# deemoe404/rmcv

Hardware: AMD Instinct MI355X
Metric: frames/sec (1280x1024 BGR) armour detect (higher is better)
Workload: dtype u8

## Files before the change

### rmcv_amd/csrc/device_fit.h

```cpp
#pragma once
#include <hip/hip_runtime.h>
#include <float.h>

#include "../../include/rmcv_abi.h"
#include "pinned_math.h"
#include "device_eig3.h"

namespace rmcv {

#define RMCV_PI 3.1415926535897932384626433832795

__device__ __forceinline__ double dabs(double x) { return __builtin_fabs(x); }
__device__ __forceinline__ double dsqrt(double x) { return ::sqrt(x); }

__device__ __forceinline__ double lane_get(double reg, int idx)
{
    const unsigned long long u = (unsigned long long)__double_as_longlong(reg);
    const unsigned lo = (unsigned)__builtin_amdgcn_readlane((int)(unsigned)u, idx);
    const unsigned hi = (unsigned)__builtin_amdgcn_readlane((int)(unsigned)(u >> 32), idx);
    return __longlong_as_double((long long)(((unsigned long long)hi << 32) | lo));
}
struct LaneRef {
    double* reg;
    int idx, lane;
// ... 384 lines not shown
    LaneMat3& V = E.V;
#else
    LaneMat3 H(lane), V(lane);
    LaneVec d(lane), e(lane);
#pragma unroll
    for (int i = 0; i < 3; i++)
#pragma unroll
        for (int j = 0; j < 3; j++) H[i][j] = M[i][j];
    eig_orthes(H, V, lane);
    eig_hqr2(H, V, d, e);
#endif
    const double d0 = d.get(0), d1 = d.get(1), d2 = d.get(2);
    int i0 = 0, i1 = 1, i2 = 2;
    double e0 = d0, e1 = d1;
    if (e0 < d1) { i0 = 1; i1 = 0; e0 = d1; e1 = d0; }
    if (e1 < d2) {
        i2 = i1;
        if (e0 < d2) { i1 = i0; i0 = 2; }
        else { i1 = 2; }
    }
    const int idx[3] = {i0, i1, i2};
#pragma unroll
    for (int i = 0; i < 3; i++) {
        eval[i] = d.get(idx[i]);
#pragma unroll
        for (int j = 0; j < 3; j++) evec[i][j] = lane_get(V.reg, 3 * j + idx[i]);
    }
}

template <int K>
__device__ __forceinline__ void jacobi_sym(LaneVec& A_, LaneVec& lam, LaneVec& V_)
{
#ifdef RMCV_JACOBI_PLAIN
    double A[K * K], V[K * K];
#pragma unroll
    for (int i = 0; i < K * K; i++) A[i] = A_.get(i);
#else
    LaneVec& A = A_;
    LaneVec& V = V_;
#endif
#pragma unroll
    for (int i = 0; i < K; i++)
#pragma unroll
        for (int j = 0; j < K; j++) V[i * K + j] = (i == j) ? 1.0 : 0.0;
#pragma unroll 1
    for (int sweep = 0; sweep < 60; sweep++) {
        double off = 0.0;
#pragma unroll
        for (int p = 0; p < K; p++)
#pragma unroll
            for (int q = p + 1; q < K; q++) off += dabs(A[p * K + q]);
        if (off == 0.0) break;
#pragma unroll
        for (int p = 0; p < K; p++)
#pragma unroll
            for (int q = p + 1; q < K; q++) {
                double apq = A[p * K + q];
                if (apq == 0.0) continue;
                double app = A[p * K + p], aqq = A[q * K + q];
                if (dabs(apq) < 1e-300 || dabs(apq) <= 1.1102230246251565e-16 * 1e-3 * dsqrt(dabs(app * aqq))) {
                    A[p * K + q] = 0.0;
                    A[q * K + p] = 0.0;
                    continue;
                }
                double theta = (aqq - app) / (2.0 * apq);
                double t = 1.0 / (dabs(theta) + dsqrt(theta * theta + 1.0));
                if (theta < 0) t = -t;
                double c = 1.0 / dsqrt(t * t + 1.0);
                double s = t * c;
                A[p * K + p] = app - t * apq;
                A[q * K + q] = aqq + t * apq;
                A[p * K + q] = 0.0;
                A[q * K + p] = 0.0;
#pragma unroll
                for (int r = 0; r < K; r++) {
                    if (r != p && r != q) {
                        double arp = A[r * K + p], arq = A[r * K + q];
                        double nrp = c * arp - s * arq;
                        double nrq = s * arp + c * arq;
                        A[r * K + p] = nrp;
                        A[p * K + r] = nrp;
                        A[r * K + q] = nrq;
                        A[q * K + r] = nrq;
                    }
                    double vrp = V[r * K + p], vrq = V[r * K + q];
                    V[r * K + p] = c * vrp - s * vrq;
                    V[r * K + q] = s * vrp + c * vrq;
                }
            }
    }
#ifdef RMCV_JACOBI_PLAIN
#pragma unroll
    for (int i = 0; i < K * K; i++) {
        A_[i] = A[i];
        V_[i] = V[i];
    }
#endif
#pragma unroll
    for (int i = 0; i < K; i++) lam[i] = (double)A[i * K + i];
}

struct NormalFac {
    LaneVec lam, V;
    int k, use;
    __device__ __forceinline__ explicit NormalFac(int lane) : lam(lane), V(lane), k(0), use(0) {}
};

template <int K>
__device__ __forceinline__ void normal_factor(LaneVec& A, NormalFac& F, double* wmax, double* wmin)
{
    F.k = K;
    jacobi_sym<K>(A, F.lam, F.V);
    double wsum = 0, mx = 0, mn = 0;
#pragma unroll
    for (int i = 0; i < K; i++) {
        const double li = F.lam[i];
        const double wi = li > 0 ? dsqrt(li) : 0.0;
        wsum += wi;
        if (i == 0 || wi > mx) mx = wi;
        if (i == 0 || wi < mn) mn = wi;
    }
    const double thr = 2.0 * DBL_EPSILON * wsum;
    F.use = 0;
#pragma unroll
    for (int i = 0; i < K; i++) {
        const double li = F.lam[i];
        const double wi = li > 0 ? dsqrt(li) : 0.0;
        F.use |= (wi > thr ? 1 : 0) << i;
    }
    *wmax = mx;
    *wmin = mn;
}
// ... 300 lines not shown
```

### rmcv_amd/csrc/k_contours.hip

```cpp
#include "contours_device.h"

namespace rmcv {

#define KC_KERNEL k_contours_w8
#define KC_THREADS 512
#include "k_contours_kernel.inc"
#undef KC_KERNEL
#undef KC_THREADS

static_assert(sizeof(ContoursLds) >= (CT_THREADS_MAX / 64) * sizeof(WaveLds), "the fit rows reuse the contour tables");

static hipError_t launch_contours_w8(const Geom& g, const Bufs& b, const Limits& lim, const SparseTail& X, int flags, const SparseSched& Q, int grid,
                                     SparseLds lds, hipStream_t s)
{
    static bool attr_set[MAX_DEVICES] = {};
    if (!attr_set[g.device]) {
        hipError_t e = hipFuncSetAttribute(reinterpret_cast<const void*>(k_contours_w8), hipFuncAttributeMaxDynamicSharedMemorySize,
                                           (int)lds_bytes(CT_MAXH));
        if (e != hipSuccess) return e;
        attr_set[g.device] = true;
    }
    return launch(k_contours_w8, dim3(grid), dim3(512), sparse_lds(lds, lds_bytes(g.h)), s, b.bits, b.rowmask, g.h, b.lab, b.neg, g.w,
                       g.h, g.ww, g.prow, g.plane_pitch, b.points, b.cont_start, b.cont_len, b.n_contours, b.n_points, b.status,
                       lim.max_contours, lim.max_points, flags, b.elig, b.n_elig, b.slot_kind, X, b.visit_xy, b.mid, b.mid_stride,
                       b.mid_slot_cap, Q, lds_rows_cap(g.h));
}

static hipError_t launch_contours_x(const Geom& g, const Bufs& b, const Limits& lim, const SparseTail& X, const RunPlan& plan, hipStream_t s,
                                    bool* lean)
{
    SparseSched Q;
    Q.order = b.frame_order;
    const SparseLaunches L = resolve_sparse({plan.form, plan.sparse_waves, X.fused != 0, X.C.enabled != 0, g.contour_tier, b.mid != nullptr,
                                             g.h <= CT_MAXH && g.ww <= 32, plan.pixel_ws != 0});
    if (lean) *lean = L.n == 1 && L.l[0].kernel == SPARSE_W_LEAN;
    for (int i = 0; i < L.n; i++) {
        const SparseLaunch& l = L.l[i];
        const hipError_t e = (l.kernel == SPARSE_W8 ? launch_contours_w8 : l.kernel == SPARSE_W4 ? launch_contours_w4 : launch_contours_lean)(
            g, b, lim, X, l.flags, Q, g.n_frames, l.lds, s);
        if (e != hipSuccess) return e;
    }
    return hipSuccess;
}

hipError_t launch_contours(const Geom& g, const Bufs& b, const Limits& lim, hipStream_t s)
{
    SparseTail X;
    memset(&X, 0, sizeof(X));
    return launch_contours_x(g, b, lim, X, RunPlan{0, 0, 8, SPARSE_STANDARD}, s, nullptr);
}

hipError_t launch_sparse(const Geom& g, const Bufs& b, const Limits& lim, const rmcv_params& p, bool pairs, bool identity, const RunPlan& plan,
                         hipStream_t s, bool* lean)
{
    SparseTail X;
    memset(&X, 0, sizeof(X));
    X.fused = 1;
    X.G = {p.tilt_max, p.ratio_lo, p.ratio_hi, p.area_lo, p.area_hi, g.overloads};
    X.slot_ell = b.slot_ell;
    FitTail& T = X.T;
    T.blobs = b.blobs;
    T.blob_src = b.blob_src;
    T.ellipses = b.ellipses;
    T.neg_idx = b.neg_idx;
    T.n_blobs = b.n_blobs;
    T.n_neg = b.n_neg;
    T.status = b.status;
    T.armours = b.armours;
    T.n_armours = b.n_armours;
    T.max_blobs = lim.max_blobs;
    T.max_armours = lim.max_armours;
    T.enemy = p.camp;
    T.enemy_tab = enemy_table(g, b);
    T.do_pairs = pairs ? 1 : 0;
    T.angle_diff_max = p.angle_diff_max;
    T.shear_max = p.shear_max;
    T.length_ratio_max = p.length_ratio_max;
    T.ov = g.overloads;
    if (identity && pairs) X.C = classify_args(g, b);
    return launch_contours_x(g, b, lim, X, plan, s, lean);
}

__device__ __forceinline__ void export_lists(const ExportArgs& a, int gtid, int nthreads)
{
    if (gtid < 12 && a.hdr_src[gtid]) a.hdr_dst[gtid] = *a.hdr_src[gtid];
    for (int k = 0; k < a.n_sec; k++) {
        const ExportSec& e = a.sec[k];
        int n = e.count ? e.count[0] + e.count_add : e.max_elems;
        n = n < 0 ? 0 : (n > e.max_elems ? e.max_elems : n);
        const int ndw = n * (e.elem_bytes >> 2);
        const uint32_t* src = static_cast<const uint32_t*>(e.src);
// ... 114 lines not shown
```

### rmcv_amd/csrc/k_contours_kernel.inc

```
#define CT_THREADS KC_THREADS
#ifndef RMCV_KC_ATTR
#define RMCV_KC_ATTR
#endif
__global__ __launch_bounds__(CT_THREADS) RMCV_KC_ATTR void KC_KERNEL(const uint64_t* __restrict__ bits, const uint32_t* __restrict__ rowmasks,
                                                        int rm_pitch, uint64_t* lab, uint64_t* neg, int w, int h, int ww, int prow,
                                                        int64_t plane_pitch, rmcv_point* points, int32_t* cont_start,
                                                        int32_t* cont_len, int32_t* n_contours, int32_t* n_points,
                                                        int32_t* status, int max_contours, int max_points, int force_literal,
                                                        int32_t* __restrict__ elig, int32_t* __restrict__ n_elig,
                                                        int32_t* __restrict__ slot_kind, SparseTail X, uint32_t* __restrict__ visit_xy,
                                                        uint8_t* __restrict__ mid_base, int64_t mid_stride, int mid_slot_cap, SparseSched Q, int rows_cap)
{
    extern __shared__ unsigned long long smem_raw[];
#ifndef RMCV_KC_PRIO
#define RMCV_KC_PRIO 3
#endif
    __builtin_amdgcn_s_setprio(RMCV_KC_PRIO);
    ContoursLds& S = *reinterpret_cast<ContoursLds*>(smem_raw);
    const RowTabs RT = row_tabs(smem_raw, rows_cap);
    const int tid = threadIdx.x, lane = tid & 63, wave = tid >> 6;
    enum { FL_COMPLEX = 1, FL_MID = 2 };
    const int f = Q.order ? Q.order[blockIdx.x] : (int)blockIdx.x;
#ifdef RMCV_PROFILE_HANDOVER
    const long long th0_ = wall_clock64(), th1_ = th0_;
#endif
    const bool defer_mid = (force_literal & 4) != 0, deferred_only = (force_literal & 8) != 0;
    force_literal &= 3;
    if (deferred_only && status[f] != RMCV_FRAME_DEFERRED_) return;
    const uint64_t* F = bits + (int64_t)f * plane_pitch;
    uint64_t* LAB = lab + (int64_t)f * plane_pitch;
    uint64_t* NEG = neg + (int64_t)f * plane_pitch;
    rmcv_point* pts = points + (int64_t)f * max_points;
    int32_t* cs = cont_start + (int64_t)f * max_contours;
// ... 220 lines not shown
    const int32_t* el = elig + (int64_t)f * max_contours;
    uint16_t* const w_len = S.n_b;
    uint16_t* const w_idx = S.n_d;
    uint16_t* const w_sorted = S.n_a;
    const uint32_t* const w_off = S.w_off;
    const uint32_t* const w_cnt = S.w_cnt;
    static_assert(KEPT_CAP <= NN_CAP, "the work list fits the node tables");
    for (int e = tid; e < ne; e += CT_THREADS) {
        int len;
        if (complex) {
            const int k = el[e];
            len = cl[k];
            w_idx[e] = (uint16_t)k;
        } else len = (int)w_cnt[e];
        w_len[e] = (uint16_t)(len > 65535 ? 65535 : len);
    }
    if (tid == 0) S.wnext = 0;
    __syncthreads();
    for (int e = tid; e < ne; e += CT_THREADS) {
        const int len = w_len[e];
        int rank = 0;
        for (int j = 0; j < ne; j++) rank += (w_len[j] > len) || (w_len[j] == len && j < e);
        w_sorted[rank] = (uint16_t)e;
    }
    __syncthreads();
    {
        static_assert(offsetof(ContoursLds, n_a) >= (CT_THREADS_MAX / 64) * sizeof(WaveLds), "the work list must outlive the tables");
        static_assert(offsetof(ContoursLds, w_off) >= (CT_THREADS_MAX / 64) * sizeof(WaveLds), "... and so must its LDS copies of starts / lengths");
        WaveLds& L = reinterpret_cast<WaveLds*>(smem_raw)[wave];
        for (;;) {
            const int got = atomicAdd(lane == 0 ? &S.wnext : &S.sink[lane], lane == 0 ? 1 : 0);
            const int e = __shfl(got, 0);
            if (e >= ne_all) break;
            if (!complex) {
                const int pos = w_sorted[e];
                fit_contour_slot_at(f, (int)w_idx[pos], nc, pts, (int)w_off[pos], (int)w_cnt[pos], max_contours, max_points, X.G, slot_kind,
                                    X.slot_ell, L, lane);
            } else {
                const int k = e < ne ? (int)w_idx[w_sorted[e]] : el[e];
                fit_contour_slot(f, k, nc, pts, cs, cl, max_contours, max_points, X.G, slot_kind, X.slot_ell, L, lane);
            }
        }
    }
    __syncthreads();
#if defined(RMCV_PROFILE) || defined(RMCV_PROFILE_HANDOVER)
    const long long tt1_ = wall_clock64();
#endif
    if (wave == 0) {
        const FitTail& T = X.T;
        const int enemy = tail_enemy(T, f);
        const int np = blob_compact_frame(f, lane, slot_kind, X.slot_ell, nc, max_contours, enemy, T.blobs, T.blob_src, T.ellipses,
                                          T.neg_idx, T.n_blobs, T.n_neg, T.status, T.max_blobs);
        if (T.do_pairs) {
            __threadfence_block();
            armours_frame(f, lane, T.blobs, np, T.max_blobs, T.angle_diff_max, T.shear_max, T.length_ratio_max, enemy, T.armours,
                          T.n_armours, T.status, T.max_armours, T.ov);
        }
    }
#ifdef RMCV_PROFILE
    __syncthreads();
    if (tid == 0 && blockIdx.x < 2) printf("[tail b%d] eligible %d of %d contours: fits %.1f us, compaction + pairing %.1f us\n", (int)blockIdx.x, ne_all, nc, (tt1_ - tt0_) / 100.0, (wall_clock64() - tt1_) / 100.0);
#endif
#ifdef RMCV_PROFILE_HANDOVER
    __syncthreads();
    if (tid == 0)
        printf("[sp] %d %lld %lld %lld | %.1f %.1f %.1f %.1f %.1f | elig %d\n", f, th0_, th1_, (long long)wall_clock64(), (t_[1] - t_[0]) / 100.0,
               (t_[2] - t_[1]) / 100.0, (tt0_ - t_[2]) / 100.0, (tt1_ - tt0_) / 100.0, (wall_clock64() - tt1_) / 100.0, ne_all);
#endif
#ifndef KC_NO_CLASSIFY
    if (X.C.enabled) {
        __threadfence_block();
        __syncthreads();
        constexpr int NW = CT_THREADS / 64;
        static_assert((CT_THREADS_MAX / 64) * sizeof(WaveLds) + NW * (NFEAT * sizeof(float) + 32 * sizeof(double)) <= sizeof(ContoursLds), "feature rows fit");
// ... 12 lines not shown
```

### rmcv_amd/csrc/k_contours_w4.hip

```cpp
#include "contours_device.h"

#include <algorithm>

namespace rmcv {

#define KC_KERNEL k_contours_w4
#define KC_THREADS 256
#include "k_contours_kernel.inc"
#undef KC_KERNEL
#undef KC_THREADS

hipError_t launch_contours_w4(const Geom& g, const Bufs& b, const Limits& lim, const SparseTail& X, int flags, const SparseSched& Q, int grid,
                              SparseLds lds, hipStream_t s)
{
    static bool attr_set[MAX_DEVICES] = {};
    if (!attr_set[g.device]) {
        hipError_t e = hipFuncSetAttribute(reinterpret_cast<const void*>(k_contours_w4), hipFuncAttributeMaxDynamicSharedMemorySize,
                                           (int)std::max(lds_bytes(CT_MAXH), LDS_ONE_PER_CU_BYTES));
        if (e != hipSuccess) return e;
        attr_set[g.device] = true;
    }
    return launch(k_contours_w4, dim3(grid), dim3(256), sparse_lds(lds, lds_bytes(g.h)), s, b.bits, b.rowmask, g.h, b.lab, b.neg, g.w,
                       g.h, g.ww, g.prow, g.plane_pitch, b.points, b.cont_start, b.cont_len, b.n_contours, b.n_points, b.status,
                       lim.max_contours, lim.max_points, flags, b.elig, b.n_elig, b.slot_kind, X, b.visit_xy, b.mid, b.mid_stride,
                       b.mid_slot_cap, Q, lds_rows_cap(g.h));
}

}
```

### rmcv_amd/csrc/k_detect.hip

```cpp
#include "device_hull.h"
#include "wave_detect.h"

namespace rmcv {

static constexpr int FIT_CHUNKS = 4;
__global__ __launch_bounds__(256) void k_fit(const rmcv_point* __restrict__ points, const int32_t* __restrict__ cont_start,
                                            const int32_t* __restrict__ cont_len, const int32_t* __restrict__ n_contours,
                                            int max_contours, int max_points, float tilt_max, float ratio_lo, float ratio_hi,
                                            double area_lo, double area_hi, int32_t* __restrict__ slot_kind,
                                            rmcv_rrect* __restrict__ slot_ell, const int32_t* __restrict__ elig,
                                            const int32_t* __restrict__ n_elig, int ov)
{
    __shared__ WaveLds lds[4];
    __builtin_amdgcn_s_setprio(3);
    const int f = blockIdx.x, lane = threadIdx.x & 63, wave = threadIdx.x >> 6;
    WaveLds& L = lds[wave];
    const int n = n_contours[f];
    const rmcv_point* pts = points + (int64_t)f * max_points;
    const int32_t* cs = cont_start + (int64_t)f * max_contours;
    const int32_t* cl = cont_len + (int64_t)f * max_contours;
    const int ne = n_elig[f];
    const FitGates G = {tilt_max, ratio_lo, ratio_hi, area_lo, area_hi, ov};
    for (int e = blockIdx.y * 4 + wave; e < ne; e += 4 * gridDim.y)
        fit_contour_slot(f, elig[(int64_t)f * max_contours + e], n, pts, cs, cl, max_contours, max_points, G, slot_kind, slot_ell, L, lane);
}

struct MatchArgs {
    float min_ratio, max_ratio, tilt_angle, min_area, max_area;
    int fit_ellipse, mode;
    int ov;
    int wcap, hcap, ccap;
    int pass;
    const uint8_t* frames;
    int64_t frame_pitch;
    int stride;
    const rmcv_point* win_eff;
};

static constexpr int MATCH_CHUNKS = 16;
static constexpr int MATCH_DEFERRED = 0x100;
__global__ __launch_bounds__(64) void k_match(const rmcv_point* __restrict__ points, const int32_t* __restrict__ cont_start,
                                             const int32_t* __restrict__ cont_len, const int32_t* __restrict__ n_contours,
                                             int max_contours, int max_points, MatchArgs A, int32_t* __restrict__ slot_kind,
                                             rmcv_rrect* __restrict__ slot_ell, const int32_t* __restrict__ elig,
                                             const int32_t* __restrict__ n_elig, int32_t* __restrict__ status)
{
    extern __shared__ unsigned long long match_smem[];
    __builtin_amdgcn_s_setprio(3);
    const int f = blockIdx.x, lane = threadIdx.x;
    WaveLds& L = *reinterpret_cast<WaveLds*>(match_smem);
    HullLds H;
    hull_lds_carve(reinterpret_cast<unsigned char*>(match_smem) + sizeof(WaveLds), A.wcap, A.hcap, A.ccap, H);
    const bool final_pass = A.pass == 1 || A.mode == 1;
    const int n = n_contours[f];
    const rmcv_point* pts = points + (int64_t)f * max_points;
    const int32_t* cs = cont_start + (int64_t)f * max_contours;
    const int32_t* cl = cont_len + (int64_t)f * max_contours;
// ... 281 lines not shown
```

### rmcv_amd/csrc/wave_detect.h

```cpp
#pragma once
#include "device_classify.h"
#include "device_fit.h"
#include "rmcv_internal.h"

namespace rmcv {

__device__ __forceinline__ int lanes_below(uint64_t m, int lane) { return __popcll(m & ((1ull << lane) - 1)); }

struct WaveLds {
    double rows[64][6];
    double terms[64];
    double dm[32];
};

__device__ __forceinline__ double wave_sum_f64(double v)
{
    for (int d = 32; d >= 1; d >>= 1) v += __shfl_xor(v, d);
    return v;
}
__device__ __forceinline__ long long wave_sum_i64(long long v)
{
    for (int d = 32; d >= 1; d >>= 1) v += __shfl_xor(v, d);
    return v;
}

template <typename F>
__device__ __forceinline__ double seq_sum_terms(int n, int lane, WaveLds& L, F term)
{
    double s = 0;
    for (int base = 0; base < n; base += 64) {
        const int i = base + lane;
        const double t = i < n ? term(i) : 0.0;
        const int m = n - base < 64 ? n - base : 64;
        if (m == 64) {
#pragma unroll
            for (int j = 0; j < 64; j++) s += lane_get(t, j);
        } else {
            for (int j = 0; j < m; j++) s += lane_get(t, j);
        }
    }
    return s;
}

template <typename F0, typename F1>
__device__ __forceinline__ void seq_sum_terms2(int n, int lane, F0 term0, F1 term1, double* s0_, double* s1_)
{
    double s0 = 0, s1 = 0;
    for (int base = 0; base < n; base += 64) {
        const int i = base + lane;
        const double t0 = i < n ? term0(i) : 0.0, t1 = i < n ? term1(i) : 0.0;
        const int m = n - base < 64 ? n - base : 64;
        if (m == 64) {
#pragma unroll
            for (int j = 0; j < 64; j++) { s0 += lane_get(t0, j); s1 += lane_get(t1, j); }
        } else {
            for (int j = 0; j < m; j++) { s0 += lane_get(t0, j); s1 += lane_get(t1, j); }
        }
    }
    *s0_ = s0;
    *s1_ = s1;
}

template <int NR, typename F>
__device__ __forceinline__ double seq_sum_products_two(int n, int lane, WaveLds& L, int ns, int la, int lb, F make_row )
{
    double acc = 0;
    const int half = lane >> 5, l5 = lane & 31;
    for (int base = 0; base < n; base += 32) {
        const int i = base + l5;
        if (i < n) {
            double r[NR];
            make_row(i, half, r);
#pragma unroll
            for (int k = 0; k < NR; k++) L.rows[lane][k] = r[k];
        }
        __builtin_amdgcn_wave_barrier();
        const int m = n - base < 32 ? n - base : 32;
        if (l5 < ns) {
            const int r0 = half * 32;
#pragma unroll 8
            for (int j = 0; j < m; j++) acc += L.rows[r0 + j][la] * L.rows[r0 + j][lb];
        }
        __builtin_amdgcn_wave_barrier();
    }
    return acc;
}

template <int NR, typename F>
__device__ __forceinline__ double seq_sum_products(int n, int lane, WaveLds& L, int ns, int la, int lb, double konst, F make_row)
{
    double acc = 0;
    for (int base = 0; base < n; base += 64) {
        const int i = base + lane;
        if (i < n) {
            double r[NR];
            make_row(i, r);
#pragma unroll
            for (int k = 0; k < NR; k++) L.rows[lane][k] = r[k];
        }
        __builtin_amdgcn_wave_barrier();
        const int m = n - base < 64 ? n - base : 64;
        if (lane < ns) {
            if (lb >= 0) {
#pragma unroll 8
                for (int j = 0; j < m; j++) acc += L.rows[j][la] * L.rows[j][lb];
            } else {
#pragma unroll 8
                for (int j = 0; j < m; j++) acc += L.rows[j][la] * konst;
            }
        }
        __builtin_amdgcn_wave_barrier();
    }
    return acc;
}

template <int K, typename F>
__device__ __forceinline__ void par_sum_products(int n, int lane, double konst, double* out, F make_row)
{
    constexpr int NT = K * (K + 1) / 2, NS = NT + K;
    double acc[NS];
#pragma unroll
    for (int e = 0; e < NS; e++) acc[e] = 0.0;
#pragma unroll 1
    for (int i = lane; i < n; i += 64) {
        double row[K];
        make_row(i, row);
        int e = 0;
#pragma unroll
        for (int a = 0; a < K; a++)
#pragma unroll
            for (int b = a; b < K; b++, e++) acc[e] += row[a] * row[b];
#pragma unroll
        for (int a = 0; a < K; a++) acc[NT + a] += row[a] * konst;
    }
    for (int d = 32; d >= 1; d >>= 1) {
        double o[NS];
#pragma unroll
        for (int e = 0; e < NS; e++) o[e] = __shfl_xor(acc[e], d);
#pragma unroll
        for (int e = 0; e < NS; e++) acc[e] += o[e];
    }
#pragma unroll
    for (int e = 0; e < NS; e++) out[e] = acc[e];
}

__device__ __forceinline__ void tri_index(int e, int k, int* a, int* b)
{
    int r = 0, rem = e;
    while (r < k && rem >= k - r) { rem -= k - r; r++; }
    *a = r;
    *b = r + rem;
}

template <int K, typename F>
__device__ __forceinline__ void normal_refine(NormalFac& Fac, int n, int lane, double bconst, double* x , F make_row)
{
    LaneVec xv(lane);
#pragma unroll
    for (int a = 0; a < K; a++) xv.reg = lane == a ? x[a] : xv.reg;
    for (int step = 0; step < 2; step++) {
        double xs[K];
#pragma unroll
        for (int a = 0; a < K; a++) xs[a] = xv.get(a);
        double acc[K];
#pragma unroll
        for (int a = 0; a < K; a++) acc[a] = 0.0;
#pragma unroll 1
        for (int i = lane; i < n; i += 64) {
            double row[K];
            make_row(i, row);
            double t = row[0] * xs[0];
#pragma unroll
            for (int b = 1; b < K; b++) t += row[b] * xs[b];
            const double r = bconst - t;
#pragma unroll
            for (int a = 0; a < K; a++) acc[a] += row[a] * r;
        }
        for (int d = 32; d >= 1; d >>= 1) {
            double o[K];
#pragma unroll
            for (int a = 0; a < K; a++) o[a] = __shfl_xor(acc[a], d);
#pragma unroll
            for (int a = 0; a < K; a++) acc[a] += o[a];
        }
        LaneVec h(lane);
#pragma unroll
        for (int a = 0; a < K; a++) h.reg = lane == a ? acc[a] : h.reg;
        double dx[5];
        normal_apply<K>(Fac, h, dx, lane);
#pragma unroll
        for (int a = 0; a < K; a++) xv.reg = lane == a ? xs[a] + dx[a] : xv.reg;
    }
#pragma unroll
    for (int a = 0; a < K; a++) x[a] = xv.get(a);
}

#ifdef RMCV_PROFILE_FITS
#define FSTAMP(k) do { if (prof) prof[k] = wall_clock64(); } while (0)
#else
#define FSTAMP(k) do {} while (0)
#endif
__device__ inline int fit_ellipse_wave(const rmcv_point* __restrict__ pts, int n, long long sumx, long long sumy, WaveLds& L, int lane,
                                rmcv_rrect* box, long long* prof = nullptr)
{
    FSTAMP(0);
    bool g_have = false;
    double g_s = 0;
    {
        const double cx = (double)sumx / n, cy = (double)sumy / n;
        g_have = sumx < (1ll << 24) && sumy < (1ll << 24);
        const float gcx = (float)sumx / (float)n, gcy = (float)sumy / (float)n;
        double s;
        if (g_have) {
            seq_sum_terms2(n, lane,
                           [&](int i) { return dabs((float)pts[i].x - cx) + dabs((float)pts[i].y - cy); },
                           [&](int i) { const float px = (float)pts[i].x - gcx, py = (float)pts[i].y - gcy; return dabs((double)px) + dabs((double)py); },
                           &s, &g_s);
        } else {
            s = seq_sum_terms(n, lane, L, [&](int i) { return dabs((float)pts[i].x - cx) + dabs((float)pts[i].y - cy); });
        }
        const double scale = 100.0 / (s > FLT_EPSILON ? s : (double)FLT_EPSILON);
        FSTAMP(1);
        int la = 0, lb = 0;
        tri_index((lane & 31) < 21 ? (lane & 31) : 0, 6, &la, &lb);
        double DM[6][6], TM[3][3], M[3][3], Ts = 0;
        const float eps1 = (float)(s / (n * 2) * 1e-2);
        const double acc = seq_sum_products_two<6>(n, lane, L, 21, la, lb, [&](int i, int set, double* r) {
            float ox, oy;
            get_ofs(i, set ? eps1 : 0.0f, &ox, &oy);
            const double px = (((float)pts[i].x + ox) - cx) * scale, py = (((float)pts[i].y + oy) - cy) * scale;
            r[0] = px * px; r[1] = px * py; r[2] = py * py; r[3] = px; r[4] = py; r[5] = 1.0;
        });
        const double inv_n = 1.0 / n;
        if ((lane & 31) < 21) (lane < 32 ? L.dm : L.terms)[lane & 31] = acc * inv_n;
        __builtin_amdgcn_wave_barrier();
        int iter;
        {
            const double* src = lane < 32 ? L.dm : L.terms;
            {
                int e = 0;
#pragma unroll
                for (int a = 0; a < 6; a++)
#pragma unroll
                    for (int b = a; b < 6; b++, e++) DM[a][b] = DM[b][a] = src[e];
            }
            const double det = direct_reduce(DM, TM, &Ts, M);
            const double det0 = lane_get(det, 0), det1 = lane_get(det, 32);
            iter = dabs(det0) > 1.0e-10 ? 0 : (dabs(det1) > 1.0e-10 ? 1 : 2);
            const int sel = iter == 1 ? 32 : 0;
#pragma unroll
            for (int a = 0; a < 3; a++)
#pragma unroll
                for (int b = 0; b < 3; b++) {
                    TM[a][b] = lane_get(TM[a][b], sel);
                    M[a][b] = lane_get(M[a][b], sel);
                }
            Ts = lane_get(Ts, sel);
        }
        __builtin_amdgcn_wave_barrier();
        FSTAMP(2);
        if (iter < 2) {
            direct_finish(M, TM, Ts, scale, cx, cy, box, lane);
            FSTAMP(3);
            if (is_good_box(box)) return 0;
        }
        FSTAMP(3);
    }
    {
        float cx, cy;
        if (sumx < (1ll << 24) && sumy < (1ll << 24)) {
            cx = (float)sumx;
            cy = (float)sumy;
        } else {
            cx = 0;
            cy = 0;
            for (int i = 0; i < n; i++) { cx += (float)pts[i].x; cy += (float)pts[i].y; }
        }
        cx /= (float)n;
        cy /= (float)n;
        const double s = g_have ? g_s : seq_sum_terms(n, lane, L, [&](int i) {
            const float px = (float)pts[i].x - cx, py = (float)pts[i].y - cy;
            return dabs((double)px) + dabs((double)py);
        });
        const double scale = 100.0 / (s > FLT_EPSILON ? s : (double)FLT_EPSILON);
        FSTAMP(8);
        double gfp[5], rp[5] = {0, 0, 0, 0, 0};
        float eps = 0.0f;
        int la = 0, lb = 0;
        if (lane < 15) tri_index(lane, 5, &la, &lb);
        else { la = lane < 20 ? lane - 15 : 0; lb = -1; }
        for (int iter = 0; iter < 2; iter++) {
            auto row5 = [&](int i, double* r) {
                float ox = 0, oy = 0;
                if (iter) get_ofs(i, eps, &ox, &oy);
                const float fx = ((float)pts[i].x + ox) - cx, fy = ((float)pts[i].y + oy) - cy;
                const double px = fx * scale, py = fy * scale;
                r[0] = -px * px; r[1] = -py * py; r[2] = -px * py; r[3] = px; r[4] = py;
            };
            {
                double sums[20];
                par_sum_products<5>(n, lane, 10000.0, sums, row5);
#pragma unroll
                for (int e = 0; e < 20; e++)
                    if (lane == e) L.dm[e] = sums[e];
            }
            __builtin_amdgcn_wave_barrier();
            LaneVec G(lane), g(lane);
            {
                const int a = lane / 5, b = lane - 5 * a;
                const int lo = a < b ? a : b, hi = a < b ? b : a;
                const int e = lo * 5 - lo * (lo - 1) / 2 + (hi - lo);
                G.reg = lane < 25 ? L.dm[e] : 0.0;
                g.reg = lane < 5 ? L.dm[15 + lane] : 0.0;
            }
            __builtin_amdgcn_wave_barrier();
            FSTAMP(9);
            NormalFac Fac(lane);
            double wmax, wmin;
            normal_factor<5>(G, Fac, &wmax, &wmin);
            FSTAMP(10);
            if (iter == 0 && wmax * FLT_EPSILON > wmin) {
                eps = (float)(s / (n * 2) * 1e-3);
                continue;
            }
            normal_apply<5>(Fac, g, gfp, lane);
            FSTAMP(11);
            normal_refine<5>(Fac, n, lane, 10000.0, gfp, row5);
            break;
        }
        FSTAMP(4);
        general_centre(gfp, rp);
        if (lane < 6) tri_index(lane, 3, &la, &lb);
        else { la = lane < 9 ? lane - 6 : 0; lb = -1; }
        const double r0 = rp[0], r1 = rp[1];
        auto row3 = [&](int i, double* r) {
            float ox = 0, oy = 0;
            if (eps != 0.0f) get_ofs(i, eps, &ox, &oy);
            const float fx = ((float)pts[i].x + ox) - cx, fy = ((float)pts[i].y + oy) - cy;
            const double px = fx * scale, py = fy * scale;
            r[0] = (px - r0) * (px - r0); r[1] = (py - r1) * (py - r1); r[2] = (px - r0) * (py - r1);
        };
        {
            double sums[9];
            par_sum_products<3>(n, lane, 1.0, sums, row3);
#pragma unroll
            for (int e = 0; e < 9; e++)
                if (lane == e) L.dm[e] = sums[e];
        }
        __builtin_amdgcn_wave_barrier();
        LaneVec G(lane), g(lane);
        {
            const int a = lane / 3, b = lane - 3 * a;
            const int lo = a < b ? a : b, hi = a < b ? b : a;
            const int e = lo * 3 - lo * (lo - 1) / 2 + (hi - lo);
            G.reg = lane < 9 ? L.dm[e] : 0.0;
            g.reg = lane < 3 ? L.dm[6 + lane] : 0.0;
        }
        __builtin_amdgcn_wave_barrier();
        FSTAMP(5);
        NormalFac Fac(lane);
        double wmax3, wmin3;
        normal_factor<3>(G, Fac, &wmax3, &wmin3);
        normal_apply<3>(Fac, g, gfp, lane);
        FSTAMP(12);
        normal_refine<3>(Fac, n, lane, 1.0, gfp, row3);
        FSTAMP(13);
        general_finish(gfp, rp, scale, cx, cy, box);
        FSTAMP(6);
    }
    return 1;
}

struct FitGates {
    float tilt_max, ratio_lo, ratio_hi;
    double area_lo, area_hi;
    int ov;
};
__device__ inline void fit_contour_slot_at(int f, int k, int n, const rmcv_point* __restrict__ pts, int start, int len, int max_contours,
                                           int max_points, const FitGates& G, int32_t* __restrict__ slot_kind,
                                           rmcv_rrect* __restrict__ slot_ell, WaveLds& L, int lane)
{
    const int c = n - 1 - k;
    int kind = 0;
    rmcv_rrect ell = {0, 0, 0, 0, 0};
    if (len >= 6 && start + len <= max_points) {
        const rmcv_point* cp = pts + start;
        double a00 = 0;
        long long sx = 0, sy = 0;
        for (int i = lane; i < len; i += 64) {
            const rmcv_point p = cp[i], q = cp[i == 0 ? len - 1 : i - 1];
            a00 += (double)(float)q.x * (float)p.y - (double)(float)q.y * (float)p.x;
            sx += p.x;
            sy += p.y;
        }
        a00 = wave_sum_f64(a00);
        sx = wave_sum_i64(sx);
        sy = wave_sum_i64(sy);
        const double area = dabs(a00 * 0.5);
        if (area >= G.area_lo && area <= G.area_hi) {
#ifdef RMCV_PROFILE_FITS
            long long pr[16] = {0, 0, 0, 0, 0, 0, 0, 0, 0, 0, 0, 0, 0, 0, 0, 0};
            const int path = fit_ellipse_wave(cp, len, sx, sy, L, lane, &ell, pr);
            if (lane == 0 && ((f == 0 && len > 150) || (path == 1 && f < 64)))
                printf("[fit f%d c%d n=%d path=%d] s %.1f moments+reduce %.1f finish %.1f | gen: s %.1f sums20 %.1f jacobi5 %.1f apply %.1f refine5 %.1f | "
                       "centre+sums9 %.1f jacobi3+apply %.1f refine3 %.1f finish %.1f us\n", f, c, len, path, (pr[1] - pr[0]) / 100.0,
                       (pr[2] - pr[1]) / 100.0, (pr[3] - pr[2]) / 100.0, (pr[8] - pr[3]) / 100.0, (pr[9] - pr[8]) / 100.0, (pr[10] - pr[9]) / 100.0,
                       (pr[11] - pr[10]) / 100.0, (pr[4] - pr[11]) / 100.0, (pr[5] - pr[4]) / 100.0, (pr[12] - pr[5]) / 100.0,
                       (pr[13] - pr[12]) / 100.0, (pr[6] - pr[13]) / 100.0);
#else
            fit_ellipse_wave(cp, len, sx, sy, L, lane, &ell);
#endif
            bool negative = false;
            const float mx = ell.w > ell.h ? ell.w : ell.h, mn = ell.w < ell.h ? ell.w : ell.h;
            const float ratio = mx / mn;
            if (!(ratio >= G.ratio_lo && ratio <= G.ratio_hi)) negative = true;
            const float angle = ell.angle > 90 ? ell.angle - 90 : ell.angle + 90;
            if (abs_ov(angle - 90, G.ov) > G.tilt_max) negative = true;
            kind = negative ? 2 : 1;
        }
    }
    if (lane == 0) {
        slot_kind[(int64_t)f * max_contours + c] = kind;
        slot_ell[(int64_t)f * max_contours + c] = ell;
    }
}

__device__ inline void fit_contour_slot(int f, int k, int n, const rmcv_point* __restrict__ pts, const int32_t* __restrict__ cs,
                                        const int32_t* __restrict__ cl, int max_contours, int max_points, const FitGates& G,
                                        int32_t* __restrict__ slot_kind, rmcv_rrect* __restrict__ slot_ell, WaveLds& L, int lane)
{
    fit_contour_slot_at(f, k, n, pts, cs[k], cl[k], max_contours, max_points, G, slot_kind, slot_ell, L, lane);
}

struct FitTail {
    rmcv_lightblob* blobs;
    int32_t* blob_src;
    rmcv_rrect* ellipses;
    int32_t* neg_idx;
    int32_t* n_blobs;
    int32_t* n_neg;
    int32_t* status;
    rmcv_armour* armours;
    int32_t* n_armours;
    int max_blobs, max_armours, enemy, do_pairs;
    float angle_diff_max, shear_max, length_ratio_max;
    int ov;
    const int32_t* enemy_tab;
};
__device__ __forceinline__ int tail_enemy(const FitTail& T, int f)
{
    return T.enemy_tab ? T.enemy_tab[f] : T.enemy;
}

__device__ inline int blob_compact_frame(int f, int lane, const int32_t* slot_kind, const rmcv_rrect* slot_ell, int n, int max_contours,
                                  int enemy, rmcv_lightblob* blobs, int32_t* blob_src, rmcv_rrect* ellipses, int32_t* neg_idx,
                                  int32_t* n_blobs, int32_t* n_neg, int32_t* status, int max_blobs)
{
    rmcv_lightblob* ob = blobs + (int64_t)f * max_blobs;
    int32_t* osrc = blob_src + (int64_t)f * max_blobs;
    rmcv_rrect* oell = ellipses + (int64_t)f * max_blobs;
    int32_t* oneg = neg_idx + (int64_t)f * max_contours;
    int np = 0, nn = 0;
    for (int base = 0; base < n; base += 64) {
        const int c = base + lane;
// ... 59 lines not shown
            const int j = i + 1 + rem;
            bool ok = false;
            rmcv_lightblob a, b;
            if (base + lane < total) {
                a = lb[i];
                b = lb[j];
                ok = a.target == enemy && b.target == enemy && pair_ok(a, b, angle_diff_max, shear_max, length_ratio_max, ov);
            }
            const uint64_t m = __ballot(ok);
            if (ok) {
                const int o = na + lanes_below(m, lane);
                if (o < max_armours) {
                    make_armour(&a, &b, &out[o], ov);
                    out[o].blob_i = i;
                    out[o].blob_j = j;
                }
            }
            na += __popcll(m);
            rem += 64;
            while (i < n - 1 && rem >= n - 1 - i) { rem -= n - 1 - i; i++; }
        }
    }
    if (lane == 0) {
        if (na > max_armours) {
            atomicOr(&status[f], RMCV_FRAME_OVF_ARMOURS);
            na = max_armours;
        }
        n_armours[f] = na;
    }
}

struct SparseTail {
    int fused;
    FitGates G;
    rmcv_rrect* slot_ell;
    FitTail T;
    ClassifyArgs C;
};

hipError_t launch_contours_w4(const Geom& g, const Bufs& b, const Limits& lim, const SparseTail& X, int flags, const SparseSched& Q, int grid,
                              SparseLds lds, hipStream_t s);
hipError_t launch_contours_lean(const Geom& g, const Bufs& b, const Limits& lim, const SparseTail& X, int flags, const SparseSched& Q, int grid, SparseLds lds,
                                hipStream_t s);

}
```

Measured before the change: 1.198 million.

## Cache contour points in packed 16-bit registers for wave ellipse fitting

Each wave now loads a contour's points once into per-lane registers, packing x and y as 16-bit halves of one word (up to 8 blocks of 64 points). The many passes of the ellipse fit (moment sums, normal equations, refinement) read points from those registers or through shuffles instead of reloading them from global memory. The w4 kernel also switches to the plain-array Jacobi path, which touches only the upper triangle of the symmetric matrix. The cost is more register pressure, which could lower occupancy, plus select chains to index the register blocks.

```diff
diff --git a/rmcv_amd/csrc/device_fit.h b/rmcv_amd/csrc/device_fit.h
--- a/rmcv_amd/csrc/device_fit.h
+++ b/rmcv_amd/csrc/device_fit.h
@@ -440,10 +440,14 @@
 __device__ __forceinline__ void jacobi_sym(LaneVec& A_, LaneVec& lam, LaneVec& V_)
 {
 #ifdef RMCV_JACOBI_PLAIN
+#define JA(i, j) A[(i) <= (j) ? (i) * K + (j) : (j) * K + (i)]
     double A[K * K], V[K * K];
 #pragma unroll
-    for (int i = 0; i < K * K; i++) A[i] = A_.get(i);
+    for (int i = 0; i < K; i++)
+#pragma unroll
+        for (int j = i; j < K; j++) JA(i, j) = A_.get(i * K + j);
 #else
+#define JA(i, j) A[(i) * K + (j)]
     LaneVec& A = A_;
     LaneVec& V = V_;
 #endif
@@ -457,18 +461,18 @@
 #pragma unroll
         for (int p = 0; p < K; p++)
 #pragma unroll
-            for (int q = p + 1; q < K; q++) off += dabs(A[p * K + q]);
+            for (int q = p + 1; q < K; q++) off += dabs(JA(p, q));
         if (off == 0.0) break;
 #pragma unroll
         for (int p = 0; p < K; p++)
 #pragma unroll
             for (int q = p + 1; q < K; q++) {
-                double apq = A[p * K + q];
+                double apq = JA(p, q);
                 if (apq == 0.0) continue;
-                double app = A[p * K + p], aqq = A[q * K + q];
+                double app = JA(p, p), aqq = JA(q, q);
                 if (dabs(apq) < 1e-300 || dabs(apq) <= 1.1102230246251565e-16 * 1e-3 * dsqrt(dabs(app * aqq))) {
-                    A[p * K + q] = 0.0;
-                    A[q * K + p] = 0.0;
+                    JA(p, q) = 0.0;
+                    JA(q, p) = 0.0;
                     continue;
                 }
                 double theta = (aqq - app) / (2.0 * apq);
@@ -476,20 +480,20 @@
                 if (theta < 0) t = -t;
                 double c = 1.0 / dsqrt(t * t + 1.0);
                 double s = t * c;
-                A[p * K + p] = app - t * apq;
-                A[q * K + q] = aqq + t * apq;
-                A[p * K + q] = 0.0;
-                A[q * K + p] = 0.0;
+                JA(p, p) = app - t * apq;
+                JA(q, q) = aqq + t * apq;
+                JA(p, q) = 0.0;
+                JA(q, p) = 0.0;
 #pragma unroll
                 for (int r = 0; r < K; r++) {
                     if (r != p && r != q) {
-                        double arp = A[r * K + p], arq = A[r * K + q];
+                        double arp = JA(r, p), arq = JA(r, q);
                         double nrp = c * arp - s * arq;
                         double nrq = s * arp + c * arq;
-                        A[r * K + p] = nrp;
-                        A[p * K + r] = nrp;
-                        A[r * K + q] = nrq;
-                        A[q * K + r] = nrq;
+                        JA(r, p) = nrp;
+                        JA(p, r) = nrp;
+                        JA(r, q) = nrq;
+                        JA(q, r) = nrq;
                     }
                     double vrp = V[r * K + p], vrq = V[r * K + q];
                     V[r * K + p] = c * vrp - s * vrq;
@@ -500,12 +504,13 @@
 #ifdef RMCV_JACOBI_PLAIN
 #pragma unroll
     for (int i = 0; i < K * K; i++) {
-        A_[i] = A[i];
+        A_[i] = JA(i / K, i % K);
         V_[i] = V[i];
     }
 #endif
 #pragma unroll
-    for (int i = 0; i < K; i++) lam[i] = (double)A[i * K + i];
+    for (int i = 0; i < K; i++) lam[i] = (double)JA(i, i);
+#undef JA
 }
 
 struct NormalFac {
diff --git a/rmcv_amd/csrc/k_contours.hip b/rmcv_amd/csrc/k_contours.hip
--- a/rmcv_amd/csrc/k_contours.hip
+++ b/rmcv_amd/csrc/k_contours.hip
@@ -4,6 +4,9 @@
 
 #define KC_KERNEL k_contours_w8
 #define KC_THREADS 512
+#ifndef KC_FIT_NB
+#define KC_FIT_NB 8
+#endif
 #include "k_contours_kernel.inc"
 #undef KC_KERNEL
 #undef KC_THREADS
@@ -56,7 +59,8 @@
     SparseTail X;
     memset(&X, 0, sizeof(X));
     X.fused = 1;
-    X.G = {p.tilt_max, p.ratio_lo, p.ratio_hi, p.area_lo, p.area_hi, g.overloads};
+    X.pts16 = g.w <= 65536 && g.h <= 65536;
+    X.G ={p.tilt_max, p.ratio_lo, p.ratio_hi, p.area_lo, p.area_hi, g.overloads};
     X.slot_ell = b.slot_ell;
     FitTail& T = X.T;
     T.blobs = b.blobs;
diff --git a/rmcv_amd/csrc/k_contours_kernel.inc b/rmcv_amd/csrc/k_contours_kernel.inc
--- a/rmcv_amd/csrc/k_contours_kernel.inc
+++ b/rmcv_amd/csrc/k_contours_kernel.inc
@@ -1,4 +1,7 @@
 #define CT_THREADS KC_THREADS
+#ifndef KC_FIT_NB
+#define KC_FIT_NB 0
+#endif
 #ifndef RMCV_KC_ATTR
 #define RMCV_KC_ATTR
 #endif
@@ -285,14 +288,18 @@
             const int got = atomicAdd(lane == 0 ? &S.wnext : &S.sink[lane], lane == 0 ? 1 : 0);
             const int e = __shfl(got, 0);
             if (e >= ne_all) break;
+            int k, start, len;
             if (!complex) {
                 const int pos = w_sorted[e];
-                fit_contour_slot_at(f, (int)w_idx[pos], nc, pts, (int)w_off[pos], (int)w_cnt[pos], max_contours, max_points, X.G, slot_kind,
-                                    X.slot_ell, L, lane);
+                k = (int)w_idx[pos];
+                start = (int)w_off[pos];
+                len = (int)w_cnt[pos];
             } else {
-                const int k = e < ne ? (int)w_idx[w_sorted[e]] : el[e];
-                fit_contour_slot(f, k, nc, pts, cs, cl, max_contours, max_points, X.G, slot_kind, X.slot_ell, L, lane);
-            }
+                k = e < ne ? (int)w_idx[w_sorted[e]] : el[e];
+                start = cs[k];
+                len = cl[k];
+            }
+            fit_contour_slot_at<KC_FIT_NB>(f, k, nc, pts, start, len, max_contours, max_points, X.G, slot_kind, X.slot_ell, L, lane, X.pts16 != 0);
         }
     }
     __syncthreads();
diff --git a/rmcv_amd/csrc/k_contours_w4.hip b/rmcv_amd/csrc/k_contours_w4.hip
--- a/rmcv_amd/csrc/k_contours_w4.hip
+++ b/rmcv_amd/csrc/k_contours_w4.hip
@@ -1,3 +1,4 @@
+#define RMCV_JACOBI_PLAIN
 #include "contours_device.h"
 
 #include <algorithm>
@@ -6,6 +7,9 @@
 
 #define KC_KERNEL k_contours_w4
 #define KC_THREADS 256
+#ifndef KC_FIT_NB
+#define KC_FIT_NB 8
+#endif
 #include "k_contours_kernel.inc"
 #undef KC_KERNEL
 #undef KC_THREADS
diff --git a/rmcv_amd/csrc/k_detect.hip b/rmcv_amd/csrc/k_detect.hip
--- a/rmcv_amd/csrc/k_detect.hip
+++ b/rmcv_amd/csrc/k_detect.hip
@@ -22,7 +22,7 @@
     const int ne = n_elig[f];
     const FitGates G = {tilt_max, ratio_lo, ratio_hi, area_lo, area_hi, ov};
     for (int e = blockIdx.y * 4 + wave; e < ne; e += 4 * gridDim.y)
-        fit_contour_slot(f, elig[(int64_t)f * max_contours + e], n, pts, cs, cl, max_contours, max_points, G, slot_kind, slot_ell, L, lane);
+        fit_contour_slot<0>(f, elig[(int64_t)f * max_contours + e], n, pts, cs, cl, max_contours, max_points, G, slot_kind, slot_ell, L, lane, false);
 }
 
 struct MatchArgs {
diff --git a/rmcv_amd/csrc/wave_detect.h b/rmcv_amd/csrc/wave_detect.h
--- a/rmcv_amd/csrc/wave_detect.h
+++ b/rmcv_amd/csrc/wave_detect.h
@@ -24,13 +24,63 @@
     return v;
 }
 
-template <typename F>
-__device__ __forceinline__ double seq_sum_terms(int n, int lane, WaveLds& L, F term)
+template <int NB>
+struct FitPts {
+    const rmcv_point* g;
+    typedef uint32_t Words __attribute__((ext_vector_type(NB > 0 ? NB : 1)));
+    Words w;
+    bool reg;
+
+    __device__ __forceinline__ void load(const rmcv_point* __restrict__ cp, int n, int lane, bool ok)
+    {
+        g = cp;
+        w = (Words)(0u);
+        reg = false;
+        if constexpr (NB > 0) {
+            reg = ok && n <= 64 * NB;
+            if (reg) {
+                int tx[NB], ty[NB];
+#pragma unroll
+                for (int b = 0; b < NB; b++) {
+                    const rmcv_point t = cp[64 * b + lane < n ? 64 * b + lane : n - 1];
+                    tx[b] = t.x;
+                    ty[b] = t.y;
+                }
+#pragma unroll
+                for (int b = 0; b < NB; b++) w[b] = 64 * b + lane < n ? ((uint32_t)tx[b] | ((uint32_t)ty[b] << 16)) : 0u;
+            }
+        }
+    }
+    __device__ __forceinline__ uint32_t block(int b) const
+    {
+        uint32_t v = w[0];
+#pragma unroll
+        for (int k = 1; k < NB; k++) v = b == k ? w[k] : v;
+        return v;
+    }
+    static __device__ __forceinline__ rmcv_point unpack(uint32_t v) { return rmcv_point{(int32_t)(v & 0xFFFFu), (int32_t)(v >> 16)}; }
+    __device__ __forceinline__ rmcv_point own(int b, int i, int n) const
+    {
+        if constexpr (NB > 0)
+            if (reg) return unpack(block(b));
+        return i < n ? g[i] : rmcv_point{0, 0};
+    }
+    __device__ __forceinline__ rmcv_point other(int b, int src, int i, int n) const
+    {
+        if constexpr (NB > 0)
+            if (reg) return unpack((uint32_t)__shfl((int)block(b), src));
+        return i < n ? g[i] : rmcv_point{0, 0};
+    }
+};
+
+template <int NB, typename F>
+__device__ __forceinline__ double seq_sum_terms(const FitPts<NB>& P, int n, int lane, WaveLds& L, F term )
 {
     double s = 0;
-    for (int base = 0; base < n; base += 64) {
+    for (int base = 0, b = 0; base < n; base += 64, b++) {
         const int i = base + lane;
-        const double t = i < n ? term(i) : 0.0;
+        const rmcv_point p = P.own(b, i, n);
+        const double t = i < n ? term(i, p) : 0.0;
         const int m = n - base < 64 ? n - base : 64;
         if (m == 64) {
 #pragma unroll
@@ -42,13 +92,14 @@
     return s;
 }
 
-template <typename F0, typename F1>
-__device__ __forceinline__ void seq_sum_terms2(int n, int lane, F0 term0, F1 term1, double* s0_, double* s1_)
+template <int NB, typename F0, typename F1>
+__device__ __forceinline__ void seq_sum_terms2(const FitPts<NB>& P, int n, int lane, F0 term0, F1 term1, double* s0_, double* s1_)
 {
     double s0 = 0, s1 = 0;
-    for (int base = 0; base < n; base += 64) {
+    for (int base = 0, b = 0; base < n; base += 64, b++) {
         const int i = base + lane;
-        const double t0 = i < n ? term0(i) : 0.0, t1 = i < n ? term1(i) : 0.0;
+        const rmcv_point p = P.own(b, i, n);
+        const double t0 = i < n ? term0(i, p) : 0.0, t1 = i < n ? term1(i, p) : 0.0;
         const int m = n - base < 64 ? n - base : 64;
         if (m == 64) {
 #pragma unroll
@@ -61,16 +112,18 @@
     *s1_ = s1;
 }
 
-template <int NR, typename F>
-__device__ __forceinline__ double seq_sum_products_two(int n, int lane, WaveLds& L, int ns, int la, int lb, F make_row )
+template <int NR, int NB, typename F>
+__device__ __forceinline__ double seq_sum_products_two(const FitPts<NB>& P, int n, int lane, WaveLds& L, int ns, int la, int lb,
+                                                       F make_row )
 {
     double acc = 0;
     const int half = lane >> 5, l5 = lane & 31;
-    for (int base = 0; base < n; base += 32) {
+    for (int base = 0, c = 0; base < n; base += 32, c++) {
         const int i = base + l5;
+        const rmcv_point p = P.other(c >> 1, (c & 1) * 32 + l5, i, n);
         if (i < n) {
             double r[NR];
-            make_row(i, half, r);
+            make_row(i, p, half, r);
 #pragma unroll
             for (int k = 0; k < NR; k++) L.rows[lane][k] = r[k];
         }
@@ -86,15 +139,17 @@
     return acc;
 }
 
-template <int NR, typename F>
-__device__ __forceinline__ double seq_sum_products(int n, int lane, WaveLds& L, int ns, int la, int lb, double konst, F make_row)
+template <int NR, int NB, typename F>
+__device__ __forceinline__ double seq_sum_products(const FitPts<NB>& P, int n, int lane, WaveLds& L, int ns, int la, int lb, double konst,
+                                                   F make_row )
 {
     double acc = 0;
-    for (int base = 0; base < n; base += 64) {
+    for (int base = 0, b = 0; base < n; base += 64, b++) {
         const int i = base + lane;
+        const rmcv_point p = P.own(b, i, n);
         if (i < n) {
             double r[NR];
-            make_row(i, r);
+            make_row(i, p, r);
 #pragma unroll
             for (int k = 0; k < NR; k++) L.rows[lane][k] = r[k];
         }
@@ -114,24 +169,28 @@
     return acc;
 }
 
-template <int K, typename F>
-__device__ __forceinline__ void par_sum_products(int n, int lane, double konst, double* out, F make_row)
+template <int K, int NB, typename F>
+__device__ __forceinline__ void par_sum_products(const FitPts<NB>& P, int n, int lane, double konst, double* out, F make_row )
 {
     constexpr int NT = K * (K + 1) / 2, NS = NT + K;
     double acc[NS];
 #pragma unroll
     for (int e = 0; e < NS; e++) acc[e] = 0.0;
 #pragma unroll 1
-    for (int i = lane; i < n; i += 64) {
-        double row[K];
-        make_row(i, row);
-        int e = 0;
-#pragma unroll
-        for (int a = 0; a < K; a++)
-#pragma unroll
-            for (int b = a; b < K; b++, e++) acc[e] += row[a] * row[b];
-#pragma unroll
-        for (int a = 0; a < K; a++) acc[NT + a] += row[a] * konst;
+    for (int base = 0, b = 0; base < n; base += 64, b++) {
+        const int i = base + lane;
+        const rmcv_point p = P.own(b, i, n);
+        if (i < n) {
+            double row[K];
+            make_row(i, p, row);
+            int e = 0;
+#pragma unroll
+            for (int a = 0; a < K; a++)
+#pragma unroll
+                for (int b2 = a; b2 < K; b2++, e++) acc[e] += row[a] * row[b2];
+#pragma unroll
+            for (int a = 0; a < K; a++) acc[NT + a] += row[a] * konst;
+        }
     }
     for (int d = 32; d >= 1; d >>= 1) {
         double o[NS];
@@ -152,8 +211,9 @@
     *b = r + rem;
 }
 
-template <int K, typename F>
-__device__ __forceinline__ void normal_refine(NormalFac& Fac, int n, int lane, double bconst, double* x , F make_row)
+template <int K, int NB, typename F>
+__device__ __forceinline__ void normal_refine(NormalFac& Fac, const FitPts<NB>& P, int n, int lane, double bconst, double* x ,
+                                              F make_row )
 {
     LaneVec xv(lane);
 #pragma unroll
@@ -166,15 +226,19 @@
 #pragma unroll
         for (int a = 0; a < K; a++) acc[a] = 0.0;
 #pragma unroll 1
-        for (int i = lane; i < n; i += 64) {
-            double row[K];
-            make_row(i, row);
-            double t = row[0] * xs[0];
-#pragma unroll
-            for (int b = 1; b < K; b++) t += row[b] * xs[b];
-            const double r = bconst - t;
-#pragma unroll
-            for (int a = 0; a < K; a++) acc[a] += row[a] * r;
+        for (int base = 0, blk = 0; base < n; base += 64, blk++) {
+            const int i = base + lane;
+            const rmcv_point p = P.own(blk, i, n);
+            if (i < n) {
+                double row[K];
+                make_row(i, p, row);
+                double t = row[0] * xs[0];
+#pragma unroll
+                for (int b = 1; b < K; b++) t += row[b] * xs[b];
+                const double r = bconst - t;
+#pragma unroll
+                for (int a = 0; a < K; a++) acc[a] += row[a] * r;
+            }
         }
         for (int d = 32; d >= 1; d >>= 1) {
             double o[K];
@@ -200,7 +264,8 @@
 #else
 #define FSTAMP(k) do {} while (0)
 #endif
-__device__ inline int fit_ellipse_wave(const rmcv_point* __restrict__ pts, int n, long long sumx, long long sumy, WaveLds& L, int lane,
+template <int NB>
+__device__ __forceinline__ int fit_ellipse_wave(const FitPts<NB>& P, int n, long long sumx, long long sumy, WaveLds& L, int lane,
                                 rmcv_rrect* box, long long* prof = nullptr)
 {
     FSTAMP(0);
@@ -212,12 +277,12 @@
         const float gcx = (float)sumx / (float)n, gcy = (float)sumy / (float)n;
         double s;
         if (g_have) {
-            seq_sum_terms2(n, lane,
-                           [&](int i) { return dabs((float)pts[i].x - cx) + dabs((float)pts[i].y - cy); },
-                           [&](int i) { const float px = (float)pts[i].x - gcx, py = (float)pts[i].y - gcy; return dabs((double)px) + dabs((double)py); },
+            seq_sum_terms2(P, n, lane,
+                           [&](int i, rmcv_point p) { return dabs((float)p.x - cx) + dabs((float)p.y - cy); },
+                           [&](int i, rmcv_point p) { const float px = (float)p.x - gcx, py = (float)p.y - gcy; return dabs((double)px) + dabs((double)py); },
                            &s, &g_s);
         } else {
-            s = seq_sum_terms(n, lane, L, [&](int i) { return dabs((float)pts[i].x - cx) + dabs((float)pts[i].y - cy); });
+            s = seq_sum_terms(P, n, lane, L, [&](int i, rmcv_point p) { return dabs((float)p.x - cx) + dabs((float)p.y - cy); });
         }
         const double scale = 100.0 / (s > FLT_EPSILON ? s : (double)FLT_EPSILON);
         FSTAMP(1);
@@ -225,10 +290,10 @@
         tri_index((lane & 31) < 21 ? (lane & 31) : 0, 6, &la, &lb);
         double DM[6][6], TM[3][3], M[3][3], Ts = 0;
         const float eps1 = (float)(s / (n * 2) * 1e-2);
-        const double acc = seq_sum_products_two<6>(n, lane, L, 21, la, lb, [&](int i, int set, double* r) {
+        const double acc = seq_sum_products_two<6>(P, n, lane, L, 21, la, lb, [&](int i, rmcv_point p, int set, double* r) {
             float ox, oy;
             get_ofs(i, set ? eps1 : 0.0f, &ox, &oy);
-            const double px = (((float)pts[i].x + ox) - cx) * scale, py = (((float)pts[i].y + oy) - cy) * scale;
+            const double px = (((float)p.x + ox) - cx) * scale, py = (((float)p.y + oy) - cy) * scale;
             r[0] = px * px; r[1] = px * py; r[2] = py * py; r[3] = px; r[4] = py; r[5] = 1.0;
         });
         const double inv_n = 1.0 / n;
@@ -274,12 +339,12 @@
         } else {
             cx = 0;
             cy = 0;
-            for (int i = 0; i < n; i++) { cx += (float)pts[i].x; cy += (float)pts[i].y; }
+            for (int i = 0; i < n; i++) { cx += (float)P.g[i].x; cy += (float)P.g[i].y; }
         }
         cx /= (float)n;
         cy /= (float)n;
-        const double s = g_have ? g_s : seq_sum_terms(n, lane, L, [&](int i) {
-            const float px = (float)pts[i].x - cx, py = (float)pts[i].y - cy;
+        const double s = g_have ? g_s : seq_sum_terms(P, n, lane, L, [&](int i, rmcv_point p) {
+            const float px = (float)p.x - cx, py = (float)p.y - cy;
             return dabs((double)px) + dabs((double)py);
         });
         const double scale = 100.0 / (s > FLT_EPSILON ? s : (double)FLT_EPSILON);
@@ -290,16 +355,16 @@
         if (lane < 15) tri_index(lane, 5, &la, &lb);
         else { la = lane < 20 ? lane - 15 : 0; lb = -1; }
         for (int iter = 0; iter < 2; iter++) {
-            auto row5 = [&](int i, double* r) {
+            auto row5 = [&](int i, rmcv_point p, double* r) {
                 float ox = 0, oy = 0;
                 if (iter) get_ofs(i, eps, &ox, &oy);
-                const float fx = ((float)pts[i].x + ox) - cx, fy = ((float)pts[i].y + oy) - cy;
+                const float fx = ((float)p.x + ox) - cx, fy = ((float)p.y + oy) - cy;
                 const double px = fx * scale, py = fy * scale;
                 r[0] = -px * px; r[1] = -py * py; r[2] = -px * py; r[3] = px; r[4] = py;
             };
             {
                 double sums[20];
-                par_sum_products<5>(n, lane, 10000.0, sums, row5);
+                par_sum_products<5>(P, n, lane, 10000.0, sums, row5);
 #pragma unroll
                 for (int e = 0; e < 20; e++)
                     if (lane == e) L.dm[e] = sums[e];
@@ -325,7 +390,7 @@
             }
             normal_apply<5>(Fac, g, gfp, lane);
             FSTAMP(11);
-            normal_refine<5>(Fac, n, lane, 10000.0, gfp, row5);
+            normal_refine<5>(Fac, P, n, lane, 10000.0, gfp, row5);
             break;
         }
         FSTAMP(4);
@@ -333,16 +398,16 @@
         if (lane < 6) tri_index(lane, 3, &la, &lb);
         else { la = lane < 9 ? lane - 6 : 0; lb = -1; }
         const double r0 = rp[0], r1 = rp[1];
-        auto row3 = [&](int i, double* r) {
+        auto row3 = [&](int i, rmcv_point p, double* r) {
             float ox = 0, oy = 0;
             if (eps != 0.0f) get_ofs(i, eps, &ox, &oy);
-            const float fx = ((float)pts[i].x + ox) - cx, fy = ((float)pts[i].y + oy) - cy;
+            const float fx = ((float)p.x + ox) - cx, fy = ((float)p.y + oy) - cy;
             const double px = fx * scale, py = fy * scale;
             r[0] = (px - r0) * (px - r0); r[1] = (py - r1) * (py - r1); r[2] = (px - r0) * (py - r1);
         };
         {
             double sums[9];
-            par_sum_products<3>(n, lane, 1.0, sums, row3);
+            par_sum_products<3>(P, n, lane, 1.0, sums, row3);
 #pragma unroll
             for (int e = 0; e < 9; e++)
                 if (lane == e) L.dm[e] = sums[e];
@@ -363,12 +428,19 @@
         normal_factor<3>(G, Fac, &wmax3, &wmin3);
         normal_apply<3>(Fac, g, gfp, lane);
         FSTAMP(12);
-        normal_refine<3>(Fac, n, lane, 1.0, gfp, row3);
+        normal_refine<3>(Fac, P, n, lane, 1.0, gfp, row3);
         FSTAMP(13);
         general_finish(gfp, rp, scale, cx, cy, box);
         FSTAMP(6);
     }
     return 1;
+}
+__device__ inline int fit_ellipse_wave(const rmcv_point* __restrict__ pts, int n, long long sumx, long long sumy, WaveLds& L, int lane,
+                                       rmcv_rrect* box)
+{
+    FitPts<0> P;
+    P.load(pts, n, lane, false);
+    return fit_ellipse_wave(P, n, sumx, sumy, L, lane, box);
 }
 
 struct FitGates {
@@ -376,23 +448,45 @@
     double area_lo, area_hi;
     int ov;
 };
-__device__ inline void fit_contour_slot_at(int f, int k, int n, const rmcv_point* __restrict__ pts, int start, int len, int max_contours,
+template <int NB>
+__device__ __forceinline__ void fit_contour_slot_at(int f, int k, int n, const rmcv_point* __restrict__ pts, int start, int len, int max_contours,
                                            int max_points, const FitGates& G, int32_t* __restrict__ slot_kind,
-                                           rmcv_rrect* __restrict__ slot_ell, WaveLds& L, int lane)
+                                           rmcv_rrect* __restrict__ slot_ell, WaveLds& L, int lane, bool pts16)
 {
     const int c = n - 1 - k;
     int kind = 0;
     rmcv_rrect ell = {0, 0, 0, 0, 0};
     if (len >= 6 && start + len <= max_points) {
         const rmcv_point* cp = pts + start;
+        FitPts<NB> P;
+        P.load(cp, len, lane, pts16);
         double a00 = 0;
         long long sx = 0, sy = 0;
-        for (int i = lane; i < len; i += 64) {
-            const rmcv_point p = cp[i], q = cp[i == 0 ? len - 1 : i - 1];
-            a00 += (double)(float)q.x * (float)p.y - (double)(float)q.y * (float)p.x;
-            sx += p.x;
-            sy += p.y;
-        }
+        bool walked = false;
+        if constexpr (NB > 0) {
+            if (P.reg) {
+                uint32_t carry = (uint32_t)__builtin_amdgcn_readlane((int)P.block((len - 1) >> 6), (len - 1) & 63);
+                for (int base = 0, b = 0; base < len; base += 64, b++) {
+                    const uint32_t cur = P.block(b);
+                    const uint32_t up = (uint32_t)__shfl_up((int)cur, 1);
+                    const rmcv_point p = P.unpack(cur), q = P.unpack(lane == 0 ? carry : up);
+                    carry = (uint32_t)__builtin_amdgcn_readlane((int)cur, 63);
+                    if (base + lane < len) {
+                        a00 += (double)(float)q.x * (float)p.y - (double)(float)q.y * (float)p.x;
+                        sx += p.x;
+                        sy += p.y;
+                    }
+                }
+                walked = true;
+            }
+        }
+        if (!walked)
+            for (int i = lane; i < len; i += 64) {
+                const rmcv_point p = cp[i], q = cp[i == 0 ? len - 1 : i - 1];
+                a00 += (double)(float)q.x * (float)p.y - (double)(float)q.y * (float)p.x;
+                sx += p.x;
+                sy += p.y;
+            }
         a00 = wave_sum_f64(a00);
         sx = wave_sum_i64(sx);
         sy = wave_sum_i64(sy);
@@ -400,7 +494,7 @@
         if (area >= G.area_lo && area <= G.area_hi) {
 #ifdef RMCV_PROFILE_FITS
             long long pr[16] = {0, 0, 0, 0, 0, 0, 0, 0, 0, 0, 0, 0, 0, 0, 0, 0};
-            const int path = fit_ellipse_wave(cp, len, sx, sy, L, lane, &ell, pr);
+            const int path = fit_ellipse_wave(P, len, sx, sy, L, lane, &ell, pr);
             if (lane == 0 && ((f == 0 && len > 150) || (path == 1 && f < 64)))
                 printf("[fit f%d c%d n=%d path=%d] s %.1f moments+reduce %.1f finish %.1f | gen: s %.1f sums20 %.1f jacobi5 %.1f apply %.1f refine5 %.1f | "
                        "centre+sums9 %.1f jacobi3+apply %.1f refine3 %.1f finish %.1f us\n", f, c, len, path, (pr[1] - pr[0]) / 100.0,
@@ -408,7 +502,7 @@
                        (pr[11] - pr[10]) / 100.0, (pr[4] - pr[11]) / 100.0, (pr[5] - pr[4]) / 100.0, (pr[12] - pr[5]) / 100.0,
                        (pr[13] - pr[12]) / 100.0, (pr[6] - pr[13]) / 100.0);
 #else
-            fit_ellipse_wave(cp, len, sx, sy, L, lane, &ell);
+            fit_ellipse_wave(P, len, sx, sy, L, lane, &ell);
 #endif
             bool negative = false;
             const float mx = ell.w > ell.h ? ell.w : ell.h, mn = ell.w < ell.h ? ell.w : ell.h;
@@ -425,11 +519,12 @@
     }
 }
 
+template <int NB>
 __device__ inline void fit_contour_slot(int f, int k, int n, const rmcv_point* __restrict__ pts, const int32_t* __restrict__ cs,
                                         const int32_t* __restrict__ cl, int max_contours, int max_points, const FitGates& G,
-                                        int32_t* __restrict__ slot_kind, rmcv_rrect* __restrict__ slot_ell, WaveLds& L, int lane)
-{
-    fit_contour_slot_at(f, k, n, pts, cs[k], cl[k], max_contours, max_points, G, slot_kind, slot_ell, L, lane);
+                                        int32_t* __restrict__ slot_kind, rmcv_rrect* __restrict__ slot_ell, WaveLds& L, int lane, bool pts16)
+{
+    fit_contour_slot_at<NB>(f, k, n, pts, cs[k], cl[k], max_contours, max_points, G, slot_kind, slot_ell, L, lane, pts16);
 }
 
 struct FitTail {
@@ -555,6 +650,7 @@
 
 struct SparseTail {
     int fused;
+    int pts16;
     FitGates G;
     rmcv_rrect* slot_ell;
     FitTail T;
```

Measured after the change: 1.204 million (median of 5 runs). No clear change (+0.4%).
